# slimgroup/SetIntersectionProjection.jl

Hardware: NVIDIA B200
Metric: parsdmm_iterations_per_second (higher is better)
Workload: dtype f32

## Files before the change

### setintersectionprojection.jl_b200/csrc/kernels.cuh

```cuda
#pragma once
#include "common.cuh"
#include "ops.cuh"

namespace sipb {

constexpr int kMaxDiag = 32;
constexpr int kMaxSets = 16;

template <typename T>
struct SpmvArgs {
  const T* R;
  i64 ld;
  int nd;
  i64 off[kMaxDiag];
  i64 N;
  i64 row0;
  i64 Nglob;
  const T* x;
  T* y;
  const T* x_lo;
  const T* x_hi;
  i64 n_lo;
  const T* tab;
  unsigned gn[3];
// ... 335 lines not shown
  }
  if (nb == (T)0) {
    st->flag = -9;
    st->done = 1;
    loop_set(lc, false);
    return;
  }
  if (nr / nb <= (T)st->tol) {
    st->flag = 0;
    st->iter = 1;
    st->done = 1;
    loop_set(lc, false);
  }
  if (st->maxit < 1) {
    st->done = 1;
    loop_set(lc, false);
  }
}
template <typename T>
__global__ void __launch_bounds__(kThreads) k_p_halo_init(i64 N, i64 halo, T* __restrict__ p, const T* __restrict__ r_lo,
                                                          const T* __restrict__ r_hi, i64 n_lo) {
  for (i64 q = (i64)blockIdx.x * blockDim.x + threadIdx.x; q < halo; q += (i64)gridDim.x * blockDim.x) {
    if (r_lo) p[q - halo] = __ldcg(r_lo + (n_lo - halo + q));
    if (r_hi) p[N + q] = __ldcg(r_hi + q);
  }
}
template <typename T>
__global__ void __launch_bounds__(kThreads) k_cg_zero_x(i64 N, T* __restrict__ x, const CgState* st) {
  if (st->flag != -9) return;
  for (i64 r = (i64)blockIdx.x * blockDim.x + threadIdx.x; r < N; r += (i64)gridDim.x * blockDim.x) x[r] = (T)0;
}

template <typename T>
__global__ void __launch_bounds__(kThreads) k_cg_xr(i64 N, T* __restrict__ x, T* __restrict__ r,
                                                    const T* __restrict__ p, const T* __restrict__ Ap,
                                                    RedScratch rs, CgState* st, const __grid_constant__ CommDev cd,
                                                    i64 halo) {
  if (st->done) return;
  constexpr int VW = Vec<T>::W;
  const double pAp = st->pAp;

  const T gamma = (T)st->rr;
  const T alpha = gamma / (T)pAp;
  const bool bad = (alpha == (T)INFINITY) || (alpha < (T)0);
  double d[1] = {0.0};
  if (!bad) {
    const i64 nvec = N / VW;
    for (i64 iv = (i64)blockIdx.x * blockDim.x + threadIdx.x; iv < nvec; iv += (i64)gridDim.x * blockDim.x) {
      const i64 row = iv * VW;
      T xv[VW], rv[VW], pv[VW], av[VW];
      vload<T>(x + row, xv);
      vload<T>(r + row, rv);
      vload<T>(p + row, pv);
      vload_stream<T>(Ap + row, av);
#pragma unroll
      for (int e = 0; e < VW; ++e) {
        xv[e] = xv[e] + alpha * pv[e];
        rv[e] = rv[e] - alpha * av[e];
        d[0] += (double)rv[e] * (double)rv[e];
      }
      vstore<T>(x + row, xv);
      vstore<T>(r + row, rv);
    }
    for (i64 row = nvec * VW + (i64)blockIdx.x * blockDim.x + threadIdx.x; row < N;
         row += (i64)gridDim.x * blockDim.x) {
      const T xv = x[row] + alpha * p[row];
      const T rv = r[row] - alpha * Ap[row];
      d[0] += (double)rv * (double)rv;
      x[row] = xv;
      r[row] = rv;
    }
  }
  bool sys = false;
  if (cd.on) {
    bool lo, hi;
    block_touches_ends(N, halo, VW, lo, hi);
    sys = lo || hi;
  }
  if (grid_sum<1>(d, rs, sys)) {
    if (bad) {
      if (threadIdx.x == 0) {
        st->flag = -2;
        st->iter = st->iter + 1;
        st->loops = st->loops + 1;
        st->relres = 0.0;
        st->done = 1;
      }
    } else if (cd.on) {
      mail_allreduce<1>(cd, d, &st->rr_new);
    } else if (threadIdx.x == 0) {
      st->rr_new = d[0];
    }
  }
}

template <typename T>
__global__ void __launch_bounds__(kThreads) k_cg_p(i64 N, const T* __restrict__ r, T* __restrict__ p,
                                                   RedScratch rs, CgState* st, const __grid_constant__ CommDev cd,
                                                   i64 halo, LoopCond lc, const T* __restrict__ r_lo,
                                                   const T* __restrict__ r_hi, i64 n_lo) {
  if (st->done) {
    if (blockIdx.x == 0 && threadIdx.x == 0) loop_set(lc, false);
    return;
  }
  constexpr int VW = Vec<T>::W;
  const double rr_new = st->rr_new;

  const T nb = (T)sqrt(st->bb);
  const T res = (T)sqrt(rr_new) / nb;
  const bool conv = res <= (T)st->tol;
  const int it = st->iter + 1;
  const bool last_it = it >= st->maxit;
  if (!conv && !last_it) {
    const T gamma = (T)st->rr;
    const T beta = (T)rr_new / gamma;
    const i64 nvec = N / VW;
    for (i64 iv = (i64)blockIdx.x * blockDim.x + threadIdx.x; iv < nvec; iv += (i64)gridDim.x * blockDim.x) {
      const i64 row = iv * VW;
      T rv[VW], pv[VW];
      vload<T>(r + row, rv);
      vload<T>(p + row, pv);
#pragma unroll
      for (int e = 0; e < VW; ++e) pv[e] = rv[e] + beta * pv[e];
      vstore<T>(p + row, pv);
    }
    for (i64 row = nvec * VW + (i64)blockIdx.x * blockDim.x + threadIdx.x; row < N;
         row += (i64)gridDim.x * blockDim.x)
      p[row] = r[row] + beta * p[row];
    if (r_lo)
      for (i64 q = (i64)blockIdx.x * blockDim.x + threadIdx.x; q < halo; q += (i64)gridDim.x * blockDim.x)
        p[q - halo] = __ldcg(r_lo + (n_lo - halo + q)) + beta * p[q - halo];
    if (r_hi)
      for (i64 q = (i64)blockIdx.x * blockDim.x + threadIdx.x; q < halo; q += (i64)gridDim.x * blockDim.x)
        p[N + q] = __ldcg(r_hi + q) + beta * p[N + q];
  }
  if (last_block_ticket(rs.counter, false) && threadIdx.x == 0) {
    st->iter = it;
    st->loops = st->loops + 1;
    st->relres = (double)res;
    if (conv) {
      st->flag = 0;
      st->done = 1;
    } else if (last_it) {
      st->flag = -1;
      st->done = 1;
    } else {
      st->rr = rr_new;
      st->rr_new = rr_new;
    }
    loop_set(lc, !(conv || last_it));
  }
}

constexpr int kRdualSets = 8;
template <typename T>
struct SetRef {
  OpDev op;
  const T* y;
  const T* l;
  const T* y_old;
  T rho;
// ... 127 lines not shown
__global__ void __launch_bounds__(kThreads) k_sparse_rdual(SparseRef<T> A, const T* __restrict__ y,
                                                           const T* __restrict__ y_old, RedScratch rs, double* out) {
  double d[1] = {0.0};
  for (i64 c = (i64)blockIdx.x * blockDim.x + threadIdx.x; c < A.cols; c += (i64)gridDim.x * blockDim.x) {
    T acc = (T)0;
    for (long long q = A.cp[c]; q < A.cp[c + 1]; ++q) {
      const int r = A.ri[q];
      acc = acc + A.vt[q] * (y[r] - y_old[r]);
    }
    d[0] += (double)acc * (double)acc;
  }
  if (grid_sum<1>(d, rs) && threadIdx.x == 0) out[0] = d[0];
}

template <typename T>
struct ProjDev {
  int kind;
  T lo, hi;
  const T* lo_vec;
  const T* hi_vec;
  const T* m;
  unsigned td[3];
  unsigned td_kofs;
  int fiber_axis;
  T rho;
  T theta;
  T scale;
  T fill;
  unsigned long long key_thr;
  int keep_all;
  int keep_none;
  const unsigned long long* tie_base;
  long long tie_chunk;
  unsigned long long quota;
  int need_ties;
};

template <typename T> __device__ __forceinline__ unsigned long long mag_key(T v);
template <> __device__ __forceinline__ unsigned long long mag_key<float>(float v) {
  return (unsigned long long)(__float_as_uint(v) & 0x7fffffffu);
}
template <> __device__ __forceinline__ unsigned long long mag_key<double>(double v) {
  return (unsigned long long)(__double_as_longlong(v) & 0x7fffffffffffffffll);
}

template <typename T> __device__ __forceinline__ T t_abs(T v);
template <> __device__ __forceinline__ float t_abs<float>(float v) { return fabsf(v); }
template <> __device__ __forceinline__ double t_abs<double>(double v) { return fabs(v); }
template <typename T> __device__ __forceinline__ T t_sign(T v) {
  return v > (T)0 ? (T)1 : (v < (T)0 ? (T)-1 : v);
}
template <typename T> __device__ __forceinline__ T t_max(T a, T b) {
  return (a != a) ? a : ((b != b) ? b : (a > b ? a : b));
}
template <typename T> __device__ __forceinline__ T t_min(T a, T b) {
  return (a != a) ? a : ((b != b) ? b : (a < b ? a : b));
}

template <typename T, int PK = -1>
__device__ __forceinline__ T proj_apply(const ProjDev<T>& P, T v, i64 r) {
  switch (PK >= 0 ? PK : P.kind) {
    case SIPB_SET_BOUNDS_SCALAR:
      return t_max<T>(P.lo, t_min<T>(v, P.hi));
    case SIPB_SET_BOUNDS_VECTOR:
      return t_max<T>(P.lo_vec[r], t_min<T>(v, P.hi_vec[r]));
    case SIPB_SET_BOUNDS_FIBER: {
// ... 33 lines not shown
      }
    default:
      return v;
  }
}

__host__ __device__ __forceinline__ bool proj_is_elementwise(int kind) {
  return kind == SIPB_SET_BOUNDS_SCALAR || kind == SIPB_SET_BOUNDS_VECTOR || kind == SIPB_SET_BOUNDS_FIBER ||
         kind == SIPB_SET_DISTANCE ||
         kind == SIPB_SET_PROX_L1;
}

constexpr int kSelBins = 2048;
constexpr int kSpecBits = 11;
constexpr int kSpecLevels = 3;
struct SpecCtx {
  unsigned int* sh;
  unsigned long long guess;
  unsigned int g0;
  unsigned int above;
};
template <typename T>
__device__ __forceinline__ void spec_hist_add(SpecCtx& sc, T v);

template <typename T>
struct ProjParams {
  T theta;
  T scale;
  T fill;
  unsigned long long key_thr;
  unsigned long long quota;
  unsigned long long count_eq;
  int keep_all, keep_none, need_ties;
};

template <typename T>
struct YlArgs {
  OpDev op;
  ProjDev<T> P;
  const ProjParams<T>* dyn;
  const T* x;
  T* y;
  T* l;
  const T* y_old;
  T* s;
  int store_s;
  int skip_v;
  const double* gate;
  double gate_tau;
  T* lhat0; T* s0; T* l0; T* y0;
  T rho, gamma;
  const T* x_old;
  double* stop_out;
  int want_feas;
  int do_sums;
  int do_snapshot;
};

template <typename T, int W> __device__ __forceinline__ void load_n(const T* p, T (&v)[W]) {
  if constexpr (W == Vec<T>::W) vload<T>(p, v);
  else {
#pragma unroll
    for (int e = 0; e < W; ++e) v[e] = p[e];
  }
}
template <typename T, int W> __device__ __forceinline__ void store_n(T* p, const T (&v)[W]) {
  if constexpr (W == Vec<T>::W) vstore<T>(p, v);
  else {
#pragma unroll
    for (int e = 0; e < W; ++e) p[e] = v[e];
  }
}

template <typename T, int MODE, bool ADAPT, int W, int PK>
__device__ __forceinline__ void yl_rows(const YlArgs<T>& a, const ProjDev<T>& P, i64 r0, double* d,
                                        SpecCtx* spec = nullptr) {
  const T rho = a.rho, gamma = a.gamma;
  const T rho1 = (T)1.0 / rho;
  const bool relaxed = !(gamma == (T)1);
  T s[W], yo[W], lo[W], yn[W], ln[W];
  if (MODE == 0 || MODE == 1) {
    if (relaxed || ADAPT) load_n<T, W>(a.y_old + r0, yo);
    load_n<T, W>(a.l + r0, lo);
    op_forward_n<T, W>(a.op, (unsigned)r0, a.x, s);
#pragma unroll
    for (int e = 0; e < W; ++e) {
      T xh = s[e];
      if (relaxed) xh = gamma * s[e] + ((T)1.0 - gamma) * yo[e];
      const T v = xh - lo[e] * rho1;
      if (MODE == 0) {
        yn[e] = proj_apply<T, PK>(P, v, r0 + e);
        const T rp = -s[e] + yn[e];
        ln[e] = relaxed ? lo[e] + rho * (-xh + yn[e]) : lo[e] + rho * rp;
        d[0] += (double)rp * (double)rp;
        if (PK != SIPB_SET_DISTANCE && a.want_feas) {
          const T pf = proj_apply<T, PK>(P, s[e], r0 + e) - s[e];
          d[1] += (double)pf * (double)pf;
          d[2] += (double)s[e] * (double)s[e];
        }
      } else {
        yn[e] = v;
        d[0] += (double)t_abs<T>(v);
        d[1] += (double)v * (double)v;
        d[2] += (v != (T)0) ? 1.0 : 0.0;
        if (spec) spec_hist_add<T>(*spec, v);
      }
    }
    if (MODE == 0 || !a.skip_v) store_n<T, W>(a.y + r0, yn);
    if (MODE == 0) store_n<T, W>(a.l + r0, ln);
    else if (a.store_s) store_n<T, W>(a.s + r0, s);
    if (MODE == 0 && PK == SIPB_SET_DISTANCE) {
      if (a.stop_out) {
        T xo[W];
        load_n<T, W>(a.x_old + r0, xo);
#pragma unroll
        for (int e = 0; e < W; ++e) {
          const T xv = s[e];
          const T dx = xo[e] - xv;
          d[1] += (double)dx * (double)dx;
          d[2] += (double)xv * (double)xv;
          const T o = xv - P.m[r0 + e];
          d[ADAPT ? 9 : 3] += (double)o * (double)o;
        }
      }
    }
  } else {
    T v[W];
    constexpr bool kRecomputeV = (PK == SIPB_SET_L1);
    if (!kRecomputeV) load_n<T, W>(a.y + r0, v);
    op_forward_n<T, W>(a.op, (unsigned)r0, a.x, s);
    load_n<T, W>(a.l + r0, lo);
    if (relaxed || ADAPT) load_n<T, W>(a.y_old + r0, yo);
#pragma unroll
    for (int e = 0; e < W; ++e) {
      if (kRecomputeV) {
        T xh = s[e];
        if (relaxed) xh = gamma * s[e] + ((T)1.0 - gamma) * yo[e];
        v[e] = xh - lo[e] * rho1;
      }
      yn[e] = proj_apply<T, PK>(P, v[e], r0 + e);
      const T rp = -s[e] + yn[e];
      if (relaxed) {
        const T xh = gamma * s[e] + ((T)1.0 - gamma) * yo[e];
        ln[e] = lo[e] + rho * (-xh + yn[e]);
      } else {
        ln[e] = lo[e] + rho * rp;
      }
      d[0] += (double)rp * (double)rp;
    }
    store_n<T, W>(a.y + r0, yn);
    store_n<T, W>(a.l + r0, ln);
  }
  if (ADAPT && MODE != 1) {
    T lh[W];
#pragma unroll
    for (int e = 0; e < W; ++e) lh[e] = lo[e] + rho * (-s[e] + yo[e]);
    if (a.do_sums) {
      T lh0[W], s0[W], l0[W], y0[W];
      load_n<T, W>(a.lhat0 + r0, lh0);
      load_n<T, W>(a.s0 + r0, s0);
      load_n<T, W>(a.l0 + r0, l0);
      load_n<T, W>(a.y0 + r0, y0);
#pragma unroll
      for (int e = 0; e < W; ++e) {
        const T dlh = lh[e] - lh0[e];
        const T dH = s[e] - s0[e];
        const T dl = ln[e] - l0[e];
        const T dG = -(yn[e] - y0[e]);
        d[3] += (double)dH * (double)dlh;
        d[4] += (double)dH * (double)dH;
        d[5] += (double)dlh * (double)dlh;
        d[6] += (double)dl * (double)dl;
        d[7] += (double)dG * (double)dG;
        d[8] += (double)dG * (double)dl;
      }
    }
    if (a.do_snapshot) {
      store_n<T, W>(a.lhat0 + r0, lh);
      store_n<T, W>(a.y0 + r0, yn);
      store_n<T, W>(a.s0 + r0, s);
      store_n<T, W>(a.l0 + r0, ln);
    }
  }
}

template <typename T, int MODE, bool ADAPT, int PK>
__device__ __forceinline__ void yl_body(const YlArgs<T>& a, const RedScratch& rs, double* out, SpecCtx* spec = nullptr) {
  constexpr int VW = Vec<T>::W;
  constexpr int NR = (ADAPT ? 9 : 3) + (MODE == 0 ? 1 : 0);
  ProjDev<T> P = a.P;
  if (a.dyn) {
    P.theta = a.dyn->theta; P.scale = a.dyn->scale; P.fill = a.dyn->fill;
    P.key_thr = a.dyn->key_thr; P.keep_all = a.dyn->keep_all; P.keep_none = a.dyn->keep_none;
    P.quota = a.dyn->quota; P.need_ties = a.dyn->need_ties;
  }
  double d[NR];
#pragma unroll
  for (int i = 0; i < NR; ++i) d[i] = 0.0;
  const i64 M = a.op.rows;
  const i64 nvec = M / VW;
  for (i64 iv = (i64)blockIdx.x * blockDim.x + threadIdx.x; iv < nvec; iv += (i64)gridDim.x * blockDim.x)
    yl_rows<T, MODE, ADAPT, VW, PK>(a, P, iv * VW, d, spec);
  for (i64 r = nvec * VW + (i64)blockIdx.x * blockDim.x + threadIdx.x; r < M; r += (i64)gridDim.x * blockDim.x)
    yl_rows<T, MODE, ADAPT, 1, PK>(a, P, r, d, spec);
  if (grid_sum<NR>(d, rs) && threadIdx.x == 0) {
    out[0] = d[0];
    if (MODE != 2) {
      out[1] = d[1];
      out[2] = d[2];
    }
    if (ADAPT) {
#pragma unroll
      for (int i = 0; i < 6; ++i) out[4 + i] = d[3 + i];
    }
    if (MODE == 0 && PK == SIPB_SET_DISTANCE && a.stop_out) {
      a.stop_out[0] = d[NR - 1];
      a.stop_out[1] = d[1];
      a.stop_out[2] = d[2];
    }
  }
}

template <typename T, int MODE, bool ADAPT>
__global__ void __launch_bounds__(kThreads, 4) k_yl(const __grid_constant__ YlArgs<T> a, RedScratch rs, double* out) {
  if (MODE == 1 && a.gate && (T)a.gate[0] <= (T)a.gate_tau) return;
  if (MODE == 2 && a.P.kind == SIPB_SET_L1) yl_body<T, MODE, ADAPT, SIPB_SET_L1>(a, rs, out);
  else yl_body<T, MODE, ADAPT, -1>(a, rs, out);
}

template <typename T>
__global__ void __launch_bounds__(kThreads, 4) k_yl_spec(const __grid_constant__ YlArgs<T> a, RedScratch rs, double* out,
                                                         unsigned long long* __restrict__ spec_above,
                                                         unsigned long long* __restrict__ spec,
                                                         const ProjParams<T>* __restrict__ guess_pp) {
  constexpr int NB = (kSpecLevels - 1) * kSelBins;
  __shared__ unsigned int sh[NB];
  __shared__ unsigned int s_above[kThreads / 32];
  for (int t = threadIdx.x; t < NB; t += blockDim.x) sh[t] = 0u;
  __syncthreads();
  const unsigned long long guess = guess_pp->key_thr;
  SpecCtx sc{sh, guess, (unsigned)(guess >> ((int)sizeof(T) * 8 - kSpecBits)), 0u};
  yl_body<T, 1, false, -1>(a, rs, out, &sc);
  unsigned int ab = sc.above;
#pragma unroll
  for (int o = 16; o > 0; o >>= 1) ab += __shfl_xor_sync(0xffffffffu, ab, o);
  if ((threadIdx.x & 31) == 0) s_above[threadIdx.x >> 5] = ab;
  __syncthreads();
  for (int t = threadIdx.x; t < NB; t += blockDim.x)
    if (sh[t]) atomicAdd(&spec[t], (unsigned long long)sh[t]);
  if (threadIdx.x == 0) {
    unsigned long long tot = 0ull;
    for (int i = 0; i < (int)(blockDim.x >> 5); ++i) tot += s_above[i];
    if (tot) atomicAdd(spec_above, tot);
  }
}

constexpr int kYlMulti = 8;
template <typename T>
struct YlMultiArgs {
// ... 604 lines not shown
```

### setintersectionprojection.jl_b200/csrc/solver.cu

```cuda
#include <algorithm>
#include <chrono>
#include <cmath>
#include <cstring>
#include <array>
#include <limits>
#include <map>
#include <memory>
#include <thread>
#include <unordered_map>
#include <vector>

#include <dlfcn.h>
#include <nccl.h>

#include "kernels.cuh"
#include <cub/device/device_radix_sort.cuh>

namespace sipb {

static thread_local std::string g_err;
void set_error(const std::string& msg) { g_err = msg; }

#define SIPB_REQUIRE(cond, code, msg)   \
  do {                                  \
// ... 403 lines not shown
    if (wl == 0) wl = st->dbits;
    if (threadIdx.x == 0)
      counts[blockIdx.x] = (unsigned long long)table[(size_t)blockIdx.x * kSelBins + (unsigned)(key & (unsigned long long)((1 << wl) - 1))];
    return;
  }
  const i64 lo = (i64)blockIdx.x * chunk, hi = min(M, lo + chunk);
  unsigned int c = 0;
  for (i64 r = lo + threadIdx.x; r < hi; r += blockDim.x) c += (mag_key<T>(v[r]) == key) ? 1u : 0u;
  __shared__ unsigned int sm[32];
  const int lane = threadIdx.x & 31, w = threadIdx.x >> 5;
#pragma unroll
  for (int o = 16; o > 0; o >>= 1) c += __shfl_xor_sync(0xffffffffu, c, o);
  if (lane == 0) sm[w] = c;
  __syncthreads();
  if (threadIdx.x == 0) {
    unsigned long long t = 0;
    for (int i = 0; i < (int)(blockDim.x >> 5); ++i) t += sm[i];
    counts[blockIdx.x] = t;
  }
}
__global__ void k_tie_totals(const unsigned long long* counts, int nblk, int g, int stride, unsigned long long* totals) {
  const int lane = threadIdx.x & 31;
  for (int b = 0; b < 4; ++b) {
    unsigned long long t = 0;
    if (b < nblk)
      for (int i = lane; i < g; i += 32) t += counts[b * stride + i];
#pragma unroll
    for (int o = 16; o > 0; o >>= 1) t += __shfl_xor_sync(0xffffffffu, t, o);
    if (lane == 0) totals[b] = t;
  }
}

template <typename T>
__global__ void __launch_bounds__(1024) k_tie_cross(i64 M, T* __restrict__ v, const ProjParams<T>* pp, i64 chunk, int g,
                                                    const unsigned long long* __restrict__ counts,
                                                    unsigned long long* __restrict__ base) {
  if (!pp->need_ties) return;
  __shared__ unsigned long long s_warp[32];
  __shared__ unsigned long long s_cross_base;
  __shared__ int s_cross;
  const unsigned long long key = pp->key_thr, quota = pp->quota;
  const int t = threadIdx.x, lane = t & 31, w = t >> 5;
  if (t == 0) s_cross = -1;
  const int per = (g + 1023) / 1024;
  unsigned long long mine = 0ull;
  for (int j = 0; j < per; ++j) {
    const int b = t * per + j;
    if (b < g) mine += counts[b];
  }
  unsigned long long incl = mine;
#pragma unroll
  for (int o = 1; o < 32; o <<= 1) {
    const unsigned long long up = __shfl_up_sync(0xffffffffu, incl, o);
    if (lane >= o) incl += up;
  }
  if (lane == 31) s_warp[w] = incl;
  __syncthreads();
  unsigned long long off = 0ull;
  for (int q = 0; q < w; ++q) off += s_warp[q];
  unsigned long long run = off + incl - mine;
  for (int j = 0; j < per; ++j) {
    const int b = t * per + j;
    if (b < g) {
      const unsigned long long nb = counts[b];
      base[b] = run;
      if (run < quota && run + nb > quota) { s_cross = b; s_cross_base = run; }
      run += nb;
    }
  }
  __syncthreads();
  const int cb = s_cross;
  if (cb < 0) return;
  const i64 lo = (i64)cb * chunk, hi = min(M, lo + chunk);
  const i64 len = (hi - lo + 1023) / 1024;
  const i64 a0 = min(hi, lo + (i64)t * len), a1 = min(hi, a0 + len);
  unsigned long long c = 0ull;
  for (i64 r = a0; r < a1; ++r) c += (mag_key<T>(v[r]) == key) ? 1ull : 0ull;
  incl = c;
#pragma unroll
  for (int o = 1; o < 32; o <<= 1) {
    const unsigned long long up = __shfl_up_sync(0xffffffffu, incl, o);
    if (lane >= o) incl += up;
  }
  __syncthreads();
  if (lane == 31) s_warp[w] = incl;
  __syncthreads();
  off = 0ull;
  for (int q = 0; q < w; ++q) off += s_warp[q];
  unsigned long long rank = s_cross_base + off + incl - c;
  if (rank + c <= quota) return;
  for (i64 r = a0; r < a1; ++r) {
    if (mag_key<T>(v[r]) == key) {
      if (rank >= quota) v[r] = (T)0;
      ++rank;
    }
  }
}

template <typename T>
__global__ void __launch_bounds__(kThreads) k_tie_zero_p(i64 M, T* __restrict__ v, const ProjParams<T>* pp, i64 chunk,
                                                         const unsigned long long* __restrict__ counts,
                                                         const unsigned long long* __restrict__ gather, int rank,
                                                         int world, int blk) {
  if (!pp->need_ties) return;
// ... 445 lines not shown
    cudaGetLastError();
    return SIPB_E_CUDA;
  }
  return SIPB_OK;
}

struct sipb_problem {
  sipb_ctx* ctx;
  int dtype;
  virtual ~sipb_problem() {}
  virtual int add_set(const sipb_set_desc* d) = 0;
  virtual int set_ata(int idx, const void* R, int64_t rows, const int64_t* offs, int nd) = 0;
  virtual int set_ata_classes(int idx, const void* tab, const int64_t* offs, int nd) = 0;
  virtual int finalize() = 0;
  virtual int solve(const void* m, void* x, void* const* l, void* const* y, const sipb_options* o, sipb_log* log) = 0;
  virtual int q_offsets(std::vector<int64_t>& out) = 0;
  virtual int q_form() const = 0;
  virtual int warm_from(sipb_problem* coarse, const sipb_resample_seg* segs, int nseg) = 0;
};

namespace sipb {

static inline double now_s() {
  return std::chrono::duration<double>(std::chrono::steady_clock::now().time_since_epoch()).count();
}

template <typename T>
struct SetT {
  sipb_set_desc desc;
  OpDev op;
  i64 M = 0;
  i64 Mglob = 0;
  DevBuf<T> y, l, y_old, s, s0, y0, l0, lhat0;
  DevBuf<T> lo_vec, hi_vec;
  DevBuf<T> perm;
  DevBuf<typename SortKey<T>::type> hkeys[2];
  DevBuf<unsigned int> hidx[2];
  DevBuf<unsigned char> hsort;
  size_t hsort_bytes = 0;
  int alloc_hist(i64 M_) {
    for (int q = 0; q < 2; ++q) {
      SIPB_CUDA_CHECK(hkeys[q].alloc((size_t)M_));
      SIPB_CUDA_CHECK(hidx[q].alloc((size_t)M_));
    }
    hsort_bytes = 0;
    SIPB_CUDA_CHECK(cub::DeviceRadixSort::SortPairs(nullptr, hsort_bytes, hkeys[0].p, hkeys[1].p, hidx[0].p, hidx[1].p, M_));
    SIPB_CUDA_CHECK(hsort.alloc(hsort_bytes + 256));
    return SIPB_OK;
  }
  SparseDev<T> sparse;
  bool is_sparse = false;
  unsigned td_kofs = 0;
  DevBuf<T> ata;
  DevBuf<T> ata_tab;
  int nd = 0;
  std::vector<int64_t> offs;
  std::vector<int> qcol;
  bool has_ata = false;
  bool tab_direct = false;
  DevBuf<ProjParams<T>> pp_y, pp_f;
  DevBuf<double> warm;
  bool z_halo = false;
  int l1_last[2] = {5, 5};
  bool l1_inactive_prev = false;
  std::map<std::array<const void*, 4>, LoopGraph> l1_graphs;
  ~SetT() { for (auto& kv : l1_graphs) kv.second.destroy(); }
// ... 145 lines not shown
    }
    SIPB_REQUIRE(minkowski ? d->block_mode != SIPB_BLOCK_PLAIN : d->block_mode == SIPB_BLOCK_PLAIN, SIPB_E_INVALID,
                 "block_mode inconsistent with the Minkowski flag of the problem");
    if (d->set_kind == SIPB_SET_L1) SIPB_REQUIRE(d->max > 0.0, SIPB_E_INVALID, "Radius of L1 ball is negative");
    if (d->set_kind == SIPB_SET_HISTOGRAM)
      SIPB_REQUIRE(!sg.on, SIPB_E_UNSUPPORTED, "the histogram set (a global sort) is single-GPU");
    auto S = std::make_unique<SetT<T>>();
    S->desc = *d;
    S->desc.sparse = nullptr;
    int rc;
    if (d->op_kind == SIPB_OP_SPARSE) {
      SIPB_REQUIRE(!sg.on && !minkowski && !fiber, SIPB_E_UNSUPPORTED,
                   "explicit sparse operators are single-GPU, non-Minkowski, matrix/tensor mode");
      SIPB_REQUIRE(d->sparse && d->sparse->cols == npts, SIPB_E_INVALID, "sparse operator must have prod(n) columns");
      rc = S->sparse.upload(d->sparse, ctx->stream);
      if (rc) return rc;
      S->is_sparse = true;
      S->op = identity_over(d->sparse->rows);
      S->M = S->op.rows;
      S->Mglob = S->M;
    } else {
      rc = make_op<T>(ndim, n, h, d->op_kind, d->block_mode, &S->op, &sg);
      if (rc) return rc;
      S->M = S->op.rows;
      S->Mglob = op_rows_host(ndim, n, d->op_kind);
    }
    S->z_halo = sg.on && op_has_slow_axis_block(S->op);
    cudaError_t e = cudaSuccess;
    auto A = [&](DevBuf<T>& b) { if (e == cudaSuccess) e = b.alloc((size_t)S->M); };
    auto AH = [&](DevBuf<T>& b) { if (e == cudaSuccess) e = b.alloc((size_t)S->M, S->z_halo ? (size_t)sg.plane : 0, 0); };
    AH(S->y); AH(S->l); AH(S->y_old); A(S->s0); A(S->y0); A(S->l0); A(S->lhat0);
    if (!proj_is_elementwise(d->set_kind) || S->is_sparse) A(S->s);
    if (d->set_kind == SIPB_SET_CARD_SLICE && d->fiber_axis != 2) A(S->perm);
    if (e == cudaSuccess) e = S->pp_y.alloc(1);
    if (e == cudaSuccess) e = S->pp_f.alloc(1);
    if (e == cudaSuccess) e = S->warm.alloc(2);
    SIPB_CUDA_CHECK(e);
    SIPB_CUDA_CHECK(cudaMemsetAsync(S->warm.p, 0, 2 * sizeof(double), ctx->stream));
    SIPB_CUDA_CHECK(cudaMemsetAsync(S->pp_y.p, 0, sizeof(ProjParams<T>), ctx->stream));
    SIPB_CUDA_CHECK(cudaMemsetAsync(S->pp_f.p, 0, sizeof(ProjParams<T>), ctx->stream));
    if (fiber) {
      SIPB_REQUIRE(d->td_n[0] * d->td_n[1] * d->td_n[2] == S->Mglob && d->td_n[0] >= 1 && d->td_n[1] >= 1 && d->td_n[2] >= 1,
                   SIPB_E_INVALID, "td_n does not match the rows of the operator");
      if (sg.on) {
        SIPB_REQUIRE(S->M % (d->td_n[0] * d->td_n[1]) == 0, SIPB_E_INVALID, "slab rows are not whole planes of td_n");
        S->desc.td_n[2] = S->M / (d->td_n[0] * d->td_n[1]);
        S->td_kofs = (unsigned)sg.k0;
      }
    }
    if (d->set_kind == SIPB_SET_HISTOGRAM) { rc = S->alloc_hist(S->M); if (rc) return rc; }
    if (d->set_kind == SIPB_SET_BOUNDS_VECTOR || d->set_kind == SIPB_SET_BOUNDS_FIBER || d->set_kind == SIPB_SET_HISTOGRAM) {
      SIPB_REQUIRE(d->min_vec && d->max_vec, SIPB_E_INVALID, "vector bounds need min_vec and max_vec");
      const size_t nb = d->set_kind == SIPB_SET_BOUNDS_FIBER ? (size_t)d->td_n[d->fiber_axis] : (size_t)S->M;
      SIPB_CUDA_CHECK(S->lo_vec.alloc(nb));
      SIPB_CUDA_CHECK(S->hi_vec.alloc(nb));
      SIPB_CUDA_CHECK(cudaMemcpyAsync(S->lo_vec.p, d->min_vec, nb * sizeof(T), cudaMemcpyHostToDevice, ctx->stream));
      SIPB_CUDA_CHECK(cudaMemcpyAsync(S->hi_vec.p, d->max_vec, nb * sizeof(T), cudaMemcpyHostToDevice, ctx->stream));
      SIPB_CUDA_CHECK(cudaStreamSynchronize(ctx->stream));
      S->desc.min_vec = S->desc.max_vec = nullptr;
    }
    maxM = std::max<i64>(maxM, S->M);
    sets.push_back(std::move(S));
    return SIPB_OK;
  }

  int set_ata(int idx, const void* R, int64_t rows, const int64_t* offs, int nd) override {
// ... 556 lines not shown
      SIPB_CUDA_CHECK(cudaMemcpyAsync(&c->d_cg->tol, &h->tol, sizeof(double), cudaMemcpyHostToDevice, c->stream));
    const bool peer = r_shared != nullptr;
    T* rr = rv();
    const CommDev& cd = peer ? c->cd_on : c->cd_off;
    T* pp = pv();
    const i64 nvecN = (N + Vec<T>::W - 1) / Vec<T>::W;
    const int g_init = c->grid_for(nvecN), g_mv = c->grid_fit((const void*)k_spmv<T, true>, nvecN),
              g_xr = c->grid_fit((const void*)k_cg_xr<T>, nvecN), g_p = c->grid_fit((const void*)k_cg_p<T>, nvecN);
    const bool tiled = tile.ok && q_classes;
    auto launch_init = [&](const LoopCond& lc) -> int {
      if (tiled) {
        const TileInit<T> ti{b, rr, pp, x_old_out};
        if ((rc = launch_tile<T, 2>(c, KC_CG_INIT, tile, false, spmv_args(xv, nullptr), ti, nullptr, nullptr, c->d_cg, cd)))
          return rc;
      } else {
        LAUNCH(c, KC_CG_INIT, k_cg_init<T>, g_init, spmv_args(xv, nullptr), b, rr, pp, x_old_out, c->rs, c->d_cg, cd);
      }
      if (!peer && (rc = c->allreduce(&c->d_cg->bb, 2))) return rc;
      LAUNCH1(c, KC_CG_FIN, k_cg_init_fin<T>, c->d_cg, cd, lc);
      if (peer)
        LAUNCH(c, KC_CG_INIT, k_p_halo_init<T>, c->grid_for(sg.plane), N, sg.plane, pp, r_lo, r_hi, n_lo);
      return SIPB_OK;
    };
    auto launch_iter = [&](const LoopCond& lc, const int* done_flag) -> int {
      if (!peer && (rc = exchange(pp, sg.nloc(), true, true))) return rc;
      if (tiled) {
        const TileInit<T> ti{nullptr, nullptr, nullptr, nullptr};
        if ((rc = launch_tile<T, 1>(c, KC_SPMV_DOT, tile, false, spmv_args_peer(Ap.p), ti, &c->d_cg->pAp, done_flag, c->d_cg, cd)))
          return rc;
      } else {
        LAUNCH(c, KC_SPMV_DOT, (k_spmv<T, true>), g_mv, spmv_args_peer(Ap.p), c->rs, &c->d_cg->pAp, done_flag, cd);
      }
      if (!peer && (rc = c->allreduce(&c->d_cg->pAp, 1))) return rc;
      LAUNCH(c, KC_CG_XR, k_cg_xr<T>, g_xr, N, xv, rr, pp, Ap.p, c->rs, c->d_cg, cd, sg.on ? sg.plane : (i64)0);
      if (!peer && (rc = c->allreduce(&c->d_cg->rr_new, 1))) return rc;
      LAUNCH(c, KC_CG_P, k_cg_p<T>, g_p, N, (const T*)rr, pp, c->rs, c->d_cg, cd, sg.on ? sg.plane : (i64)0, lc,
             peer ? r_lo : (const T*)nullptr, peer ? r_hi : (const T*)nullptr, n_lo);
      return SIPB_OK;
    };
    const double vecN = (double)N * sizeof(T);
    const double q_rows = q_classes ? 0.0 : (double)q_offs.size();
    c->account(KC_CG_INIT, (q_rows + 4 + (x_old_out ? 1 : 0)) * vecN);
    if (deferred) {
      if (!cg_graph.exec || cg_graph_key[0] != (const void*)b || cg_graph_key[1] != (const void*)xv ||
          cg_graph_key[2] != (const void*)x_old_out) {
        rc = build_loop_graph(
            c, cg_graph, [&](const LoopCond& lc) { return launch_init(lc); },
            [&](const LoopCond& lc) { return launch_iter(lc, (const int*)nullptr); },
            [&]() {
              LAUNCH(c, KC_FILL, k_cg_zero_x<T>, c->grid_for(N), N, xv, (const CgState*)c->d_cg);
              return SIPB_OK;
            });
        if (rc) { set_error("could not build the CG loop graph"); return rc; }
        cg_graph_key[0] = b; cg_graph_key[1] = xv; cg_graph_key[2] = x_old_out;
      }
      SIPB_CUDA_CHECK(cudaGraphLaunch(cg_graph.exec, c->stream));
      c->total_launches += 1;
      if ((rc = exchange(xv, sg.nloc(), true, true))) return rc;
      *deferred = true;
      return SIPB_OK;
    }
    const LoopCond off{0, 0};
    if ((rc = launch_init(off))) return rc;
    int launched = 0;
    int batch = std::max(1, predicted);
    for (;;) {
      for (int q = 0; q < batch && launched < max_iter; ++q, ++launched)
        if ((rc = launch_iter(off, (const int*)&c->d_cg->done))) return rc;
      SIPB_CUDA_CHECK(cudaMemcpyAsync(h, c->d_cg, sizeof(CgState), cudaMemcpyDeviceToHost, c->stream));
      if (peer) SIPB_CUDA_CHECK(cudaMemcpyAsync(c->h_p2p_err, c->d_p2p_err, sizeof(int), cudaMemcpyDeviceToHost, c->stream));
      SIPB_CUDA_CHECK(cudaStreamSynchronize(c->stream));
      if (peer) SIPB_REQUIRE(*c->h_p2p_err == 0, SIPB_E_NCCL, "peer-memory collective timed out (a rank stopped participating)");
      if (h->done || launched >= max_iter) break;
      batch = std::max(2, launched / 2);
    }
    account_cg_loops(h);
    if (h->flag == -9) SIPB_CUDA_CHECK(cudaMemsetAsync(xv, 0, N * sizeof(T), c->stream));
    if ((rc = exchange(xv, sg.nloc(), true, true))) return rc;
    *iters = h->iter;
    *relres = h->relres;
    *flag = h->flag;
    return SIPB_OK;
  }
  void account_cg_loops(const CgState* h) {
    sipb_ctx* c = ctx;
    const double vecN = (double)N * sizeof(T);
    const double q_rows = q_classes ? 0.0 : (double)q_offs.size();
    c->account(KC_SPMV_DOT, h->loops * (q_rows + 2) * vecN);
    c->account(KC_CG_XR, h->loops * 6 * vecN);
    c->account(KC_CG_P, std::max(0, h->loops - (h->flag == 0 ? 1 : 0)) * 3 * vecN);
  }
  void finish_cg(int* iters, double* relres, int* flag) {
    sipb_ctx* c = ctx;
    const CgState* h = c->h_cg;
    account_cg_loops(h);
    c->launches[KC_SPMV_DOT] += h->loops; c->launches[KC_CG_XR] += h->loops; c->launches[KC_CG_P] += h->loops;
    c->launches[KC_CG_INIT] += 1; c->launches[KC_CG_FIN] += 1;
    c->total_launches += 3 * (int64_t)h->loops + 2;
    *iters = h->iter;
    *relres = h->relres;
    *flag = h->flag;
  }

  int solve(const void* m_h, void* x_h, void* const* l_h, void* const* y_h, const sipb_options* o,
            sipb_log* log) override;
};

template <typename T>
static void adapt_scalar(const double* sm, T& rho, T& gamma, bool adjust_rho, bool adjust_gamma) {
  const T safeguard = (sizeof(T) == 8) ? (T)1e-10 : (T)1e-6f;
  const T eps_corr = (T)0.3;
  const T d_dHh_dlh = (T)sm[0];
  const T n_dH = (T)std::sqrt(sm[1]);
  const T n_dlh = (T)std::sqrt(sm[2]);
  const T n_dl = (T)std::sqrt(sm[3]);
  const T n_dG = (T)std::sqrt(sm[4]);
  const T d_dGh_dl = (T)sm[5];
  bool alpha_rel = false, beta_rel = false;
  T alpha_corr = 0, beta_corr = 0;
  if ((n_dH * n_dlh) > safeguard && (n_dH * n_dH) > safeguard && d_dHh_dlh > safeguard) {
    alpha_rel = true;
    alpha_corr = d_dHh_dlh / (n_dH * n_dlh);
  }
// ... 261 lines not shown
        else
          LAUNCH(c, KC_RHS, (k_rhs<T, false>), g_rhs, ra, c->rs, (double*)nullptr);
        first = false;
        s0 = s1;
      }
    }
    phase_end(1);
    int cg_it = 0, cg_flag = 0;
    double cg_relres = 0.0;
    bool cg_deferred = false;
    {
      const bool loop_on_device = c->graph_loops && !c->profile && (!sg.on || r_shared != nullptr);
      int rc = run_cg(rhs.p, x.p, x_old.p, i, 0.0, 1000, last_cg + 1, &cg_it, &cg_relres, &cg_flag,
                      loop_on_device ? &cg_deferred : nullptr);
      if (rc) return rc;
      last_cg = cg_it;
    }
    log->cg_it[i - 1] = cg_it;
    log->cg_relres[i - 1] = cg_relres;
    phase_end(2);
    const bool feas_it = (i % 10 == 0);
    const bool do_adapt = (adjust_rho || adjust_gamma) && (i % rho_update_frequency == 0);
    const bool fuse_adapt = (i == 1) || do_adapt;
    YlMultiArgs<T>& ym = yl_multi;
    int n_multi = 0, g_multi = 1;
    auto flush_multi = [&]() {
      if (n_multi == 0) return;
      const dim3 grid((unsigned)g_multi, (unsigned)n_multi);
      if (fuse_adapt) LAUNCH(c, KC_YL_FUSED, (k_yl_multi<T, true>), grid, ym, c->rs_multi);
      else LAUNCH(c, KC_YL_FUSED, (k_yl_multi<T, false>), grid, ym, c->rs_multi);
      n_multi = 0;
      g_multi = 1;
    };
    for (int s = 0; s < p; ++s) {
      SetT<T>& S = *sets[s];
      const bool is_dist = S.desc.set_kind == SIPB_SET_DISTANCE;
      const bool want_feas = feas_it && !is_dist;
      S.y.swap(S.y_old);
      YlArgs<T> ya;
      memset(&ya, 0, sizeof(ya));
      ya.op = S.op;
      ya.P = proj_static(S, rho[s]);
      ya.x = x.p; ya.y = S.y.p; ya.l = S.l.p; ya.y_old = S.y_old.p; ya.s = S.s.p;
      if (S.is_sparse) {
        LAUNCH(c, KC_OP_APPLY, k_sparse_forward<T>, c->grid_for(S.M), S.sparse.ref(), (const T*)x.p, S.s.p);
        ya.x = S.s.p;
      }
      ya.lhat0 = S.lhat0.p; ya.s0 = S.s0.p; ya.l0 = S.l0.p; ya.y0 = S.y0.p;
      ya.rho = rho[s]; ya.gamma = gamma[s];
      ya.do_sums = (do_adapt && i > 1) ? 1 : 0;
      ya.do_snapshot = fuse_adapt ? 1 : 0;
      const int base = s * kSlotPerSet;
      const i64 nvecM = (S.M + Vec<T>::W - 1) / Vec<T>::W;
      const int g = proj_is_elementwise(S.desc.set_kind)
                        ? (fuse_adapt ? c->grid_fit((const void*)k_yl_multi<T, true>, nvecM)
                                      : c->grid_fit((const void*)k_yl_multi<T, false>, nvecM))
                        : c->grid_for(nvecM);
      const double rowsB = (double)S.M * sizeof(T), colsB = (double)N * sizeof(T);
      const bool needs_yold = fuse_adapt || !(gamma[s] == (T)1);
      const double adaptB = (fuse_adapt ? 4 : 0) * rowsB + (ya.do_sums ? 4 : 0) * rowsB;
      if (proj_is_elementwise(S.desc.set_kind)) {
        if (fuse_stop && is_dist) {
          ya.x_old = x_old.p;
          ya.stop_out = c->d_scal + kSlotGlobal;
        }
        c->account(KC_YL_FUSED, colsB + (3 + (needs_yold ? 1 : 0) + (ya.stop_out ? 1 : 0)) * rowsB + adaptB);
        ya.want_feas = want_feas ? 1 : 0;
        ym.a[n_multi] = ya;
        ym.out[n_multi] = c->d_scal + base;
        g_multi = std::max(g_multi, g);
        if (++n_multi == kYlMulti) flush_multi();
      } else {
        ya.want_feas = 0;
        ya.store_s = (want_feas && !S.is_sparse) ? 1 : 0;
        const bool spec = S.desc.set_kind == SIPB_SET_CARDINALITY && !sg.on && c->sel_spec;
        if (S.desc.set_kind == SIPB_SET_L1 && !sg.on && (c->l1_skipv == 2 || (c->l1_skipv == 1 && S.l1_inactive_prev)))
          ya.skip_v = 1;
        if (spec)
          LAUNCH(c, KC_YL_PASS1, (k_yl_spec<T>), c->grid_fit((const void*)k_yl_spec<T>, nvecM), ya, c->rs,
                 c->d_scal + base + 10, &c->d_sel->spec_above, c->d_sel->spec, (const ProjParams<T>*)S.pp_y.p);
        else
          LAUNCH(c, KC_YL_PASS1, (k_yl<T, 1, false>), c->grid_fit((const void*)k_yl<T, 1, false>, nvecM), ya, c->rs,
                 c->d_scal + base + 10);
        if (ya.skip_v) {
          YlArgs<T> yb = ya;
          yb.skip_v = 0;
          yb.store_s = 0;
          yb.gate = c->d_scal + base + 10;
          yb.gate_tau = (double)(T)S.desc.max;
          LAUNCH(c, KC_YL_PASS1, (k_yl<T, 1, false>), c->grid_fit((const void*)k_yl<T, 1, false>, nvecM), yb, c->rs,
                 c->d_scal + base + 13);
        }
        const int l1set = S.desc.set_kind == SIPB_SET_L1 ? 1 : 0;
        c->account(KC_YL_PASS1, colsB + (2 - ya.skip_v + (!(gamma[s] == (T)1) ? 1 : 0) + ya.store_s) * rowsB);
        c->account(KC_YL_PASS2, colsB + (4 - l1set + (needs_yold ? 1 : 0)) * rowsB + adaptB);
        i64 tie_chunk = 0;
        const bool defer = S.desc.set_kind == SIPB_SET_CARDINALITY && !sg.on && c->sel_spec;
        int rc = projector_params(S, S.y.p, base + 10, S.pp_y.p, S.warm.p, true, spec, defer ? &tie_chunk : nullptr);
        if (rc) return rc;
        ya.dyn = S.pp_y.p;
        if (tie_chunk > 0) { ya.P.tie_base = c->d_tie_base; ya.P.tie_chunk = tie_chunk; }
        if (fuse_adapt)
          LAUNCH(c, KC_YL_PASS2, (k_yl<T, 2, true>), c->grid_fit((const void*)k_yl<T, 2, true>, nvecM), ya, c->rs,
                 c->d_scal + base);
        else
          LAUNCH(c, KC_YL_PASS2, (k_yl<T, 2, false>), c->grid_fit((const void*)k_yl<T, 2, false>, nvecM), ya, c->rs,
                 c->d_scal + base);
        if (want_feas) {
          rc = feasibility_of(S, S.s.p, base + 1, true);
          if (rc) return rc;
        }
      }
    }
    flush_multi();
    if (!fuse_rdual) {
      for (int s = 0; s < p; ++s) {
        SetT<T>& S = *sets[s];
        if (S.is_sparse)
          LAUNCH(c, KC_RDUAL, k_sparse_rdual<T>, c->grid_for(N), S.sparse.ref(), (const T*)S.y.p, (const T*)S.y_old.p, c->rs,
                 c->d_scal + s * kSlotPerSet + 3);
        else
          LAUNCH(c, KC_RDUAL, k_rdual<T>, c->grid_for((npts + Vec<T>::W - 1) / Vec<T>::W), S.op, (const T*)S.y.p,
                 (const T*)S.y_old.p, c->rs, c->d_scal + s * kSlotPerSet + 3);
      }
    }
    { int rc = exchange_yl_halos(); if (rc) return rc; }
    if (!fuse_stop) {
      LAUNCH(c, KC_STOP, k_stop<T>, c->grid_for((N + Vec<T>::W - 1) / Vec<T>::W), N, npts, minkowski ? 1 : 0, (const T*)x.p,
             (const T*)x_old.p, (const T*)m.p, c->rs, c->d_scal + kSlotGlobal);
      c->account(KC_STOP, 3.0 * N * sizeof(T));
    }
    { int rc = ctx_sync_scalars(c, true); if (rc) return rc; }
    if (c->p2p) SIPB_REQUIRE(*c->h_p2p_err == 0, SIPB_E_NCCL, "peer-memory collective timed out (a rank stopped participating)");
    SIPB_REQUIRE(!c->h_l1->failed, SIPB_E_STATE, "l1 threshold search did not converge");
    if (cg_deferred) {
      finish_cg(&cg_it, &cg_relres, &cg_flag);
      last_cg = cg_it;
      log->cg_it[i - 1] = cg_it;
      log->cg_relres[i - 1] = cg_relres;
    }
    {
      T rp_tot = 0, rd_tot = 0;
      for (int s = 0; s < p; ++s) {
        const int base = s * kSlotPerSet;
        const T rp = (T)std::sqrt(c->h_scal[base + 0]);
        LG(log->r_pri, i - 1, s, p_log) = (double)rp;
        if (sets[s]->desc.set_kind == SIPB_SET_L1 && !sg.on)
          sets[s]->l1_inactive_prev = (T)c->h_scal[base + 10] <= (T)sets[s]->desc.max;
        rp_tot = rp_tot + rp;
        if (!fuse_rdual) {
          const T rd = rho[s] * (T)std::sqrt(c->h_scal[base + 3]);
          LG(log->r_dual, i - 1, s, p_log) = (double)rd;
          rd_tot = rd_tot + rd;
        }
        if (feas_it && s < pp) {
          const T num = (T)std::sqrt(c->h_scal[base + 1]);
          const T den = (T)std::sqrt(c->h_scal[base + 2]);
          LG(log->set_feasibility, counter - 1, s, pp) = (double)(num / (den + eps100));
        }
      }
      if (feas_it) counter += 1;
      if (!fuse_rdual) {
        log->r_dual_total[i - 1] = (double)rd_tot;
      } else if (i >= 2) {
        T tot = 0;
        for (int s = 0; s < p; ++s) {
          const T rd = (T)LG(log->rho, i - 2, s, p_log) * (T)std::sqrt(c->h_scal[kSlotGlobal + 8 + s]);
          LG(log->r_dual, i - 2, s, p_log) = (double)rd;
          tot = tot + rd;
        }
        log->r_dual_total[i - 2] = (double)tot;
      }
      log->r_pri_total[i - 1] = (double)rp_tot;
      const double* g = c->h_scal + kSlotGlobal;
      const T nxm = (T)std::sqrt(g[0]);
      log->obj[i - 1] = (double)((T)0.5 * (nxm * nxm));
      log->evol_x[i - 1] = (double)((T)std::sqrt(g[1]) / (T)std::sqrt(g[2]));
      for (int s = 0; s < p; ++s) {
        LG(log->rho, i - 1, s, p_log) = (double)rho[s];
        LG(log->gamma, i - 1, s, p_log) = (double)gamma[s];
      }
// ... 1004 lines not shown
```

Measured before the change: 47.78.

## Defer CG x update into p kernel, add one-pass L1 y/l mode, recompute cardinality v

The CG x += alpha*p update moves from the x/r kernel into the p-update kernel, where it shares the load of p. That removes one full read of p and a read/write of x from the residual pass. For L1 sets with skip_v, a new MODE 3 kernel computes y, a double-buffered l, and the primal residual in a single pass. The second pass is then gated on the L1 norm, so it is skipped when the set is inactive, and the l buffers are swapped afterwards. The cardinality pass 2 now recomputes v instead of loading it, reading y only for elements on the tie boundary chunk, which adds a tie_cross field and more kernel-variant complexity.

Measured after the change: 51.10 (median of 6 runs). +6.9%, better.

```diff
diff --git a/setintersectionprojection.jl_b200/csrc/kernels.cuh b/setintersectionprojection.jl_b200/csrc/kernels.cuh
--- a/setintersectionprojection.jl_b200/csrc/kernels.cuh
+++ b/setintersectionprojection.jl_b200/csrc/kernels.cuh
@@ -391,8 +391,7 @@
 }
 
 template <typename T>
-__global__ void __launch_bounds__(kThreads) k_cg_xr(i64 N, T* __restrict__ x, T* __restrict__ r,
-                                                    const T* __restrict__ p, const T* __restrict__ Ap,
+__global__ void __launch_bounds__(kThreads) k_cg_xr(i64 N, T* __restrict__ r, const T* __restrict__ Ap,
                                                     RedScratch rs, CgState* st, const __grid_constant__ CommDev cd,
                                                     i64 halo) {
   if (st->done) return;
@@ -407,26 +406,20 @@
     const i64 nvec = N / VW;
     for (i64 iv = (i64)blockIdx.x * blockDim.x + threadIdx.x; iv < nvec; iv += (i64)gridDim.x * blockDim.x) {
       const i64 row = iv * VW;
-      T xv[VW], rv[VW], pv[VW], av[VW];
-      vload<T>(x + row, xv);
+      T rv[VW], av[VW];
       vload<T>(r + row, rv);
-      vload<T>(p + row, pv);
       vload_stream<T>(Ap + row, av);
 #pragma unroll
       for (int e = 0; e < VW; ++e) {
-        xv[e] = xv[e] + alpha * pv[e];
         rv[e] = rv[e] - alpha * av[e];
         d[0] += (double)rv[e] * (double)rv[e];
       }
-      vstore<T>(x + row, xv);
       vstore<T>(r + row, rv);
     }
     for (i64 row = nvec * VW + (i64)blockIdx.x * blockDim.x + threadIdx.x; row < N;
          row += (i64)gridDim.x * blockDim.x) {
-      const T xv = x[row] + alpha * p[row];
       const T rv = r[row] - alpha * Ap[row];
       d[0] += (double)rv * (double)rv;
-      x[row] = xv;
       r[row] = rv;
     }
   }
@@ -454,7 +447,7 @@
 }
 
 template <typename T>
-__global__ void __launch_bounds__(kThreads) k_cg_p(i64 N, const T* __restrict__ r, T* __restrict__ p,
+__global__ void __launch_bounds__(kThreads) k_cg_p(i64 N, T* __restrict__ x, const T* __restrict__ r, T* __restrict__ p,
                                                    RedScratch rs, CgState* st, const __grid_constant__ CommDev cd,
                                                    i64 halo, LoopCond lc, const T* __restrict__ r_lo,
                                                    const T* __restrict__ r_hi, i64 n_lo) {
@@ -470,22 +463,44 @@
   const bool conv = res <= (T)st->tol;
   const int it = st->iter + 1;
   const bool last_it = it >= st->maxit;
-  if (!conv && !last_it) {
-    const T gamma = (T)st->rr;
-    const T beta = (T)rr_new / gamma;
-    const i64 nvec = N / VW;
+  const T gamma = (T)st->rr;
+  const T alpha = gamma / (T)st->pAp;
+  const i64 nvec = N / VW;
+  if (conv || last_it) {
     for (i64 iv = (i64)blockIdx.x * blockDim.x + threadIdx.x; iv < nvec; iv += (i64)gridDim.x * blockDim.x) {
       const i64 row = iv * VW;
-      T rv[VW], pv[VW];
+      T xv[VW], pv[VW];
+      vload<T>(x + row, xv);
+      vload<T>(p + row, pv);
+#pragma unroll
+      for (int e = 0; e < VW; ++e) xv[e] = xv[e] + alpha * pv[e];
+      vstore<T>(x + row, xv);
+    }
+    for (i64 row = nvec * VW + (i64)blockIdx.x * blockDim.x + threadIdx.x; row < N;
+         row += (i64)gridDim.x * blockDim.x)
+      x[row] = x[row] + alpha * p[row];
+  } else {
+    const T beta = (T)rr_new / gamma;
+    for (i64 iv = (i64)blockIdx.x * blockDim.x + threadIdx.x; iv < nvec; iv += (i64)gridDim.x * blockDim.x) {
+      const i64 row = iv * VW;
+      T xv[VW], rv[VW], pv[VW];
+      vload<T>(x + row, xv);
       vload<T>(r + row, rv);
       vload<T>(p + row, pv);
 #pragma unroll
-      for (int e = 0; e < VW; ++e) pv[e] = rv[e] + beta * pv[e];
+      for (int e = 0; e < VW; ++e) {
+        xv[e] = xv[e] + alpha * pv[e];
+        pv[e] = rv[e] + beta * pv[e];
+      }
+      vstore<T>(x + row, xv);
       vstore<T>(p + row, pv);
     }
     for (i64 row = nvec * VW + (i64)blockIdx.x * blockDim.x + threadIdx.x; row < N;
-         row += (i64)gridDim.x * blockDim.x)
-      p[row] = r[row] + beta * p[row];
+         row += (i64)gridDim.x * blockDim.x) {
+      const T pv = p[row];
+      x[row] = x[row] + alpha * pv;
+      p[row] = r[row] + beta * pv;
+    }
     if (r_lo)
       for (i64 q = (i64)blockIdx.x * blockDim.x + threadIdx.x; q < halo; q += (i64)gridDim.x * blockDim.x)
         p[q - halo] = __ldcg(r_lo + (n_lo - halo + q)) + beta * p[q - halo];
@@ -679,6 +694,7 @@
   int keep_none;
   const unsigned long long* tie_base;
   long long tie_chunk;
+  long long tie_cross;
   unsigned long long quota;
   int need_ties;
 };
@@ -778,6 +794,7 @@
   unsigned long long quota;
   unsigned long long count_eq;
   int keep_all, keep_none, need_ties;
+  long long tie_cross;
 };
 
 template <typename T>
@@ -788,6 +805,8 @@
   const T* x;
   T* y;
   T* l;
+  T* l_new;
+  double* rp_out;
   const T* y_old;
   T* s;
   int store_s;
@@ -825,7 +844,7 @@
   const T rho1 = (T)1.0 / rho;
   const bool relaxed = !(gamma == (T)1);
   T s[W], yo[W], lo[W], yn[W], ln[W];
-  if (MODE == 0 || MODE == 1) {
+  if (MODE != 2) {
     if (relaxed || ADAPT) load_n<T, W>(a.y_old + r0, yo);
     load_n<T, W>(a.l + r0, lo);
     op_forward_n<T, W>(a.op, (unsigned)r0, a.x, s);
@@ -850,11 +869,17 @@
         d[1] += (double)v * (double)v;
         d[2] += (v != (T)0) ? 1.0 : 0.0;
         if (spec) spec_hist_add<T>(*spec, v);
-      }
-    }
-    if (MODE == 0 || !a.skip_v) store_n<T, W>(a.y + r0, yn);
+        if (MODE == 3) {
+          const T rp = -s[e] + yn[e];
+          ln[e] = relaxed ? lo[e] + rho * (-xh + yn[e]) : lo[e] + rho * rp;
+          d[3] += (double)rp * (double)rp;
+        }
+      }
+    }
+    if (MODE != 1 || !a.skip_v) store_n<T, W>(a.y + r0, yn);
     if (MODE == 0) store_n<T, W>(a.l + r0, ln);
-    else if (a.store_s) store_n<T, W>(a.s + r0, s);
+    if (MODE == 3) store_n<T, W>(a.l_new + r0, ln);
+    if (MODE != 0 && a.store_s) store_n<T, W>(a.s + r0, s);
     if (MODE == 0 && PK == SIPB_SET_DISTANCE) {
       if (a.stop_out) {
         T xo[W];
@@ -872,7 +897,7 @@
     }
   } else {
     T v[W];
-    constexpr bool kRecomputeV = (PK == SIPB_SET_L1);
+    constexpr bool kRecomputeV = (PK == SIPB_SET_L1 || PK == SIPB_SET_CARDINALITY);
     if (!kRecomputeV) load_n<T, W>(a.y + r0, v);
     op_forward_n<T, W>(a.op, (unsigned)r0, a.x, s);
     load_n<T, W>(a.l + r0, lo);
@@ -883,6 +908,8 @@
         T xh = s[e];
         if (relaxed) xh = gamma * s[e] + ((T)1.0 - gamma) * yo[e];
         v[e] = xh - lo[e] * rho1;
+        if (PK == SIPB_SET_CARDINALITY && mag_key<T>(v[e]) == P.key_thr && (r0 + e) / P.tie_chunk == P.tie_cross)
+          v[e] = a.y[r0 + e];
       }
       yn[e] = proj_apply<T, PK>(P, v[e], r0 + e);
       const T rp = -s[e] + yn[e];
@@ -895,9 +922,9 @@
       d[0] += (double)rp * (double)rp;
     }
     store_n<T, W>(a.y + r0, yn);
-    store_n<T, W>(a.l + r0, ln);
-  }
-  if (ADAPT && MODE != 1) {
+    store_n<T, W>((a.l_new ? a.l_new : a.l) + r0, ln);
+  }
+  if (ADAPT && (MODE == 0 || MODE == 2)) {
     T lh[W];
 #pragma unroll
     for (int e = 0; e < W; ++e) lh[e] = lo[e] + rho * (-s[e] + yo[e]);
@@ -933,12 +960,12 @@
 template <typename T, int MODE, bool ADAPT, int PK>
 __device__ __forceinline__ void yl_body(const YlArgs<T>& a, const RedScratch& rs, double* out, SpecCtx* spec = nullptr) {
   constexpr int VW = Vec<T>::W;
-  constexpr int NR = (ADAPT ? 9 : 3) + (MODE == 0 ? 1 : 0);
+  constexpr int NR = (ADAPT ? 9 : 3) + (MODE == 0 || MODE == 3 ? 1 : 0);
   ProjDev<T> P = a.P;
   if (a.dyn) {
     P.theta = a.dyn->theta; P.scale = a.dyn->scale; P.fill = a.dyn->fill;
     P.key_thr = a.dyn->key_thr; P.keep_all = a.dyn->keep_all; P.keep_none = a.dyn->keep_none;
-    P.quota = a.dyn->quota; P.need_ties = a.dyn->need_ties;
+    P.quota = a.dyn->quota; P.need_ties = a.dyn->need_ties; P.tie_cross = a.dyn->tie_cross;
   }
   double d[NR];
 #pragma unroll
@@ -955,6 +982,7 @@
       out[1] = d[1];
       out[2] = d[2];
     }
+    if (MODE == 3) a.rp_out[0] = d[3];
     if (ADAPT) {
 #pragma unroll
       for (int i = 0; i < 6; ++i) out[4 + i] = d[3 + i];
@@ -969,8 +997,9 @@
 
 template <typename T, int MODE, bool ADAPT>
 __global__ void __launch_bounds__(kThreads, 4) k_yl(const __grid_constant__ YlArgs<T> a, RedScratch rs, double* out) {
-  if (MODE == 1 && a.gate && (T)a.gate[0] <= (T)a.gate_tau) return;
+  if (MODE != 3 && a.gate && (T)a.gate[0] <= (T)a.gate_tau) return;
   if (MODE == 2 && a.P.kind == SIPB_SET_L1) yl_body<T, MODE, ADAPT, SIPB_SET_L1>(a, rs, out);
+  else if (MODE == 2 && !ADAPT && a.P.kind == SIPB_SET_CARDINALITY && a.P.tie_base) yl_body<T, MODE, ADAPT, SIPB_SET_CARDINALITY>(a, rs, out);
   else yl_body<T, MODE, ADAPT, -1>(a, rs, out);
 }
 
diff --git a/setintersectionprojection.jl_b200/csrc/solver.cu b/setintersectionprojection.jl_b200/csrc/solver.cu
--- a/setintersectionprojection.jl_b200/csrc/solver.cu
+++ b/setintersectionprojection.jl_b200/csrc/solver.cu
@@ -459,10 +459,13 @@
 }
 
 template <typename T>
-__global__ void __launch_bounds__(1024) k_tie_cross(i64 M, T* __restrict__ v, const ProjParams<T>* pp, i64 chunk, int g,
+__global__ void __launch_bounds__(1024) k_tie_cross(i64 M, T* __restrict__ v, ProjParams<T>* pp, i64 chunk, int g,
                                                     const unsigned long long* __restrict__ counts,
                                                     unsigned long long* __restrict__ base) {
-  if (!pp->need_ties) return;
+  if (!pp->need_ties) {
+    if (threadIdx.x == 0) pp->tie_cross = -1;
+    return;
+  }
   __shared__ unsigned long long s_warp[32];
   __shared__ unsigned long long s_cross_base;
   __shared__ int s_cross;
@@ -497,6 +500,7 @@
   }
   __syncthreads();
   const int cb = s_cross;
+  if (t == 0) pp->tie_cross = cb;
   if (cb < 0) return;
   const i64 lo = (i64)cb * chunk, hi = min(M, lo + chunk);
   const i64 len = (hi - lo + 1023) / 1024;
@@ -1008,6 +1012,7 @@
   i64 M = 0;
   i64 Mglob = 0;
   DevBuf<T> y, l, y_old, s, s0, y0, l0, lhat0;
+  DevBuf<T> l_alt;
   DevBuf<T> lo_vec, hi_vec;
   DevBuf<T> perm;
   DevBuf<typename SortKey<T>::type> hkeys[2];
@@ -1219,6 +1224,7 @@
     AH(S->y); AH(S->l); AH(S->y_old); A(S->s0); A(S->y0); A(S->l0); A(S->lhat0);
     if (!proj_is_elementwise(d->set_kind) || S->is_sparse) A(S->s);
     if (d->set_kind == SIPB_SET_CARD_SLICE && d->fiber_axis != 2) A(S->perm);
+    if (d->set_kind == SIPB_SET_L1 && !sg.on) A(S->l_alt);
     if (e == cudaSuccess) e = S->pp_y.alloc(1);
     if (e == cudaSuccess) e = S->pp_f.alloc(1);
     if (e == cudaSuccess) e = S->warm.alloc(2);
@@ -1841,9 +1847,9 @@
         LAUNCH(c, KC_SPMV_DOT, (k_spmv<T, true>), g_mv, spmv_args_peer(Ap.p), c->rs, &c->d_cg->pAp, done_flag, cd);
       }
       if (!peer && (rc = c->allreduce(&c->d_cg->pAp, 1))) return rc;
-      LAUNCH(c, KC_CG_XR, k_cg_xr<T>, g_xr, N, xv, rr, pp, Ap.p, c->rs, c->d_cg, cd, sg.on ? sg.plane : (i64)0);
+      LAUNCH(c, KC_CG_XR, k_cg_xr<T>, g_xr, N, rr, (const T*)Ap.p, c->rs, c->d_cg, cd, sg.on ? sg.plane : (i64)0);
       if (!peer && (rc = c->allreduce(&c->d_cg->rr_new, 1))) return rc;
-      LAUNCH(c, KC_CG_P, k_cg_p<T>, g_p, N, (const T*)rr, pp, c->rs, c->d_cg, cd, sg.on ? sg.plane : (i64)0, lc,
+      LAUNCH(c, KC_CG_P, k_cg_p<T>, g_p, N, xv, (const T*)rr, pp, c->rs, c->d_cg, cd, sg.on ? sg.plane : (i64)0, lc,
              peer ? r_lo : (const T*)nullptr, peer ? r_hi : (const T*)nullptr, n_lo);
       return SIPB_OK;
     };
@@ -1896,8 +1902,9 @@
     const double vecN = (double)N * sizeof(T);
     const double q_rows = q_classes ? 0.0 : (double)q_offs.size();
     c->account(KC_SPMV_DOT, h->loops * (q_rows + 2) * vecN);
-    c->account(KC_CG_XR, h->loops * 6 * vecN);
-    c->account(KC_CG_P, std::max(0, h->loops - (h->flag == 0 ? 1 : 0)) * 3 * vecN);
+    c->account(KC_CG_XR, h->loops * 3 * vecN);
+    const int p_loops = std::max(0, h->loops - 1);
+    c->account(KC_CG_P, (p_loops * 5 + (h->loops > 0 && h->flag != -2 ? 3 : 0)) * vecN);
   }
   void finish_cg(int* iters, double* relres, int* flag) {
     sipb_ctx* c = ctx;
@@ -2225,6 +2232,7 @@
       n_multi = 0;
       g_multi = 1;
     };
+    std::vector<double> gated_pass2B(p, 0.0);
     for (int s = 0; s < p; ++s) {
       SetT<T>& S = *sets[s];
       const bool is_dist = S.desc.set_kind == SIPB_SET_DISTANCE;
@@ -2269,13 +2277,20 @@
         const bool spec = S.desc.set_kind == SIPB_SET_CARDINALITY && !sg.on && c->sel_spec;
         if (S.desc.set_kind == SIPB_SET_L1 && !sg.on && (c->l1_skipv == 2 || (c->l1_skipv == 1 && S.l1_inactive_prev)))
           ya.skip_v = 1;
-        if (spec)
+        const int g1 = c->grid_fit((const void*)k_yl<T, 1, false>, nvecM), g2 = c->grid_fit((const void*)k_yl<T, 2, false>, nvecM);
+        const bool one_pass = ya.skip_v && !fuse_adapt && S.l_alt.p && g1 == g2;
+        if (one_pass) {
+          ya.l_new = S.l_alt.p;
+          ya.rp_out = c->d_scal + base;
+          LAUNCH(c, KC_YL_PASS1, (k_yl<T, 3, false>), g1, ya, c->rs, c->d_scal + base + 10);
+        } else if (spec) {
           LAUNCH(c, KC_YL_PASS1, (k_yl_spec<T>), c->grid_fit((const void*)k_yl_spec<T>, nvecM), ya, c->rs,
                  c->d_scal + base + 10, &c->d_sel->spec_above, c->d_sel->spec, (const ProjParams<T>*)S.pp_y.p);
-        else
+        } else {
           LAUNCH(c, KC_YL_PASS1, (k_yl<T, 1, false>), c->grid_fit((const void*)k_yl<T, 1, false>, nvecM), ya, c->rs,
                  c->d_scal + base + 10);
-        if (ya.skip_v) {
+        }
+        if (ya.skip_v && !one_pass) {
           YlArgs<T> yb = ya;
           yb.skip_v = 0;
           yb.store_s = 0;
@@ -2284,15 +2299,21 @@
           LAUNCH(c, KC_YL_PASS1, (k_yl<T, 1, false>), c->grid_fit((const void*)k_yl<T, 1, false>, nvecM), yb, c->rs,
                  c->d_scal + base + 13);
         }
-        const int l1set = S.desc.set_kind == SIPB_SET_L1 ? 1 : 0;
+        const bool defer = S.desc.set_kind == SIPB_SET_CARDINALITY && !sg.on && c->sel_spec;
+        const int recompute_v = (S.desc.set_kind == SIPB_SET_L1 || (defer && !fuse_adapt)) ? 1 : 0;
         c->account(KC_YL_PASS1, colsB + (2 - ya.skip_v + (!(gamma[s] == (T)1) ? 1 : 0) + ya.store_s) * rowsB);
-        c->account(KC_YL_PASS2, colsB + (4 - l1set + (needs_yold ? 1 : 0)) * rowsB + adaptB);
+        const double pass2B = colsB + (4 - recompute_v + (needs_yold ? 1 : 0)) * rowsB + adaptB;
+        if (one_pass) gated_pass2B[s] = pass2B;
+        c->account(KC_YL_PASS2, one_pass ? 2 * rowsB : pass2B);
         i64 tie_chunk = 0;
-        const bool defer = S.desc.set_kind == SIPB_SET_CARDINALITY && !sg.on && c->sel_spec;
         int rc = projector_params(S, S.y.p, base + 10, S.pp_y.p, S.warm.p, true, spec, defer ? &tie_chunk : nullptr);
         if (rc) return rc;
         ya.dyn = S.pp_y.p;
         if (tie_chunk > 0) { ya.P.tie_base = c->d_tie_base; ya.P.tie_chunk = tie_chunk; }
+        if (one_pass) {
+          ya.gate = c->d_scal + base + 10;
+          ya.gate_tau = (double)(T)S.desc.max;
+        }
         if (fuse_adapt)
           LAUNCH(c, KC_YL_PASS2, (k_yl<T, 2, true>), c->grid_fit((const void*)k_yl<T, 2, true>, nvecM), ya, c->rs,
                  c->d_scal + base);
@@ -2303,6 +2324,7 @@
           rc = feasibility_of(S, S.s.p, base + 1, true);
           if (rc) return rc;
         }
+        if (one_pass) S.l.swap(S.l_alt);
       }
     }
     flush_multi();
@@ -2338,8 +2360,10 @@
         const int base = s * kSlotPerSet;
         const T rp = (T)std::sqrt(c->h_scal[base + 0]);
         LG(log->r_pri, i - 1, s, p_log) = (double)rp;
-        if (sets[s]->desc.set_kind == SIPB_SET_L1 && !sg.on)
+        if (sets[s]->desc.set_kind == SIPB_SET_L1 && !sg.on) {
           sets[s]->l1_inactive_prev = (T)c->h_scal[base + 10] <= (T)sets[s]->desc.max;
+          if (!sets[s]->l1_inactive_prev) c->account(KC_YL_PASS2, gated_pass2B[s]);
+        }
         rp_tot = rp_tot + rp;
         if (!fuse_rdual) {
           const T rd = rho[s] * (T)std::sqrt(c->h_scal[base + 3]);
```
